# opherlieber/rltime

Hardware: AMD Instinct MI355X
Metric: sampled transitions/sec (= learner steps/sec x B x T), IQN-LSTM B=512 T=80 84x84x4 (higher is better)
Workload: dtype f32

## Files before the change

include/mirl.h:

```cpp
#ifndef MIRL_H
#define MIRL_H

#include <stdint.h>

#ifdef __cplusplus
extern "C" {
#endif

#define MIRL_OK 0
#define MIRL_NEED_MORE 1
#define MIRL_ERR_ARG (-1)
#define MIRL_ERR_HIP (-2)
#define MIRL_ERR_STATE (-3)
#define MIRL_ERR_NOGPU (-4)

#define MIRL_MODE_UNIFORM 0
#define MIRL_MODE_PER 1

typedef struct mirl_replay mirl_replay;

typedef struct mirl_replay_config {
  int64_t size;
  int32_t num_envs;
  int32_t env_base;
// ... 124 lines not shown
                      double gamma, double vf_eps, float* targets, void* stream);

int mirl_loss_dqn(int64_t M, int32_t A, const float* q, const int64_t* actions,
                  const float* targets, const float* weights, double kappa, int32_t mode,
                  double row_scale, float* row_loss, float* dq, float* td, void* stream);
int mirl_loss_iqn(int64_t M, int32_t N, int32_t Nt, int32_t A, const float* z,
                  const float* taus, const int64_t* actions, const float* targets,
                  const float* weights, double kappa, double row_scale,
                  float* row_loss, float* dz, float* abs_td, void* stream);

int mirl_q_target_c51(int64_t M, int32_t A, int32_t Z, const float* logits_target, const float* logits_select,
                      const float* support, const float* returns, const float* nsteps, const float* masks,
                      double gamma, double vmin, double vmax, double delta_z, int32_t projection,
                      float* targets, void* stream);
int mirl_loss_c51(int64_t M, int32_t A, int32_t Z, const float* logits, const int64_t* actions,
                  const float* targets, const float* weights, int32_t mode, double kappa, double row_scale,
                  float* row_loss, float* dlogits, float* report, void* stream);

int mirl_lstm_cell_fwd(int32_t B, int32_t H, float* gates, const float* c_in, const float* keep_next,
                       float* h_out, float* c_out, float* h_next, float* c_next, void* stream);
int mirl_lstm_seq_supported(int32_t T, int32_t B, int32_t H);
int mirl_lstm_seq_workspace_bytes(int32_t B, int32_t H, int64_t* bytes);
int mirl_lstm_seq_fwd(int32_t T, int32_t B, int32_t H, float* gx, const float* w_hh, const float* h0,
                      const float* c0, const float* keep, float* out, float* c_all, float* hm, float* cm,
                      float* h_last, float* c_last, int32_t save_gates, void* workspace, void* stream);
int mirl_lstm_seq_status(int32_t* status);
int mirl_lstm_seq_fwd_grid(int32_t B, int32_t H, int32_t* workgroups, int64_t* lds_bytes, int32_t* compute_units,
                           int32_t* per_compute_unit);
int mirl_lstm_seq_bwd_supported(int32_t T, int32_t B, int32_t H);
int mirl_lstm_seq_bwd_workspace_bytes(int32_t B, int32_t H, int64_t* bytes);
int mirl_lstm_seq_bwd(int32_t T, int32_t B, int32_t H, float* gates, const float* w_hh, const float* c_all,
                      const float* cm, const float* d_out, const float* keep, void* workspace, void* stream);
int mirl_lstm_cell_bwd(int32_t B, int32_t H, float* gates, const float* c_t, const float* c_in,
                       const float* d_out, const float* dh_rec, float* dc_rec, const float* keep_next,
                       int32_t first, void* stream);

int mirl_frames_to_f32_nhwc(int64_t N, int32_t C, int32_t HW, const uint8_t* src, float scale,
                            float* dst, void* stream);
int mirl_frames_to_f32_nhwc_ex(int64_t N, int32_t C, int32_t HW, const uint8_t* src, float scale,
                               float* dst, int32_t per_wg, int32_t flags, void* stream);

int mirl_conv1_u8_supported(int32_t C, int32_t H, int32_t W, int32_t F, int32_t K, int32_t S);
int mirl_conv1_u8_wpk_floats(int64_t* out);
int mirl_conv1_bf16_set(int32_t mode);
int mirl_conv1_wrw_bf16_set(int32_t mode);
int mirl_conv1_u8_fwd(int64_t N, int32_t H, int32_t W, const uint8_t* x, const float* weight,
                      int64_t ws_o, int64_t ws_c, int64_t ws_h, int64_t ws_w, const float* bias,
                      float scale, float* wpk, float* y, void* stream);
int mirl_conv1_u8_fwd_ex(int64_t N, int32_t H, int32_t W, const uint8_t* x, const float* weight,
                         int64_t ws_o, int64_t ws_c, int64_t ws_h, int64_t ws_w, const float* bias,
                         float scale, float* wpk, float* y, int32_t flags, void* stream);

int mirl_conv1_u8_wrw_scratch_floats(int64_t* out);
int mirl_conv1_u8_wrw(int64_t N, int32_t H, int32_t W, const uint8_t* x, const float* g, float scale,
                      float* scratch, float* dw, int64_t ws_o, int64_t ws_c, int64_t ws_h, int64_t ws_w,
                      void* stream);
int mirl_conv1_u8_wrw_ex(int64_t N, int32_t H, int32_t W, const uint8_t* x, const float* g, float scale,
                         float* scratch, float* dw, int64_t ws_o, int64_t ws_c, int64_t ws_h, int64_t ws_w,
                         int32_t flags, void* stream);
int mirl_conv1_u8_wrw_masked(int64_t N, int32_t H, int32_t W, const uint8_t* x, const float* dy, const float* y, float scale,
                             float* scratch, float* dw, int64_t ws_o, int64_t ws_c, int64_t ws_h, int64_t ws_w,
                             float* db, void* stream);

int mirl_conv2_bwd_data_supported(int32_t C, int32_t F, int32_t K, int32_t S, int32_t IH, int32_t IW,
                                  int32_t OH, int32_t OW);
int mirl_conv2_bwd_data(int64_t N, int32_t OH, int32_t OW, const float* g, const float* weight,
                        int64_t ws_o, int64_t ws_c, int64_t ws_h, int64_t ws_w, float* wpk, float* dx,
                        void* stream);
int mirl_conv2_bwd_data_wpk_floats(int64_t* floats);
int mirl_conv2_bwd_data_ex(int64_t N, int32_t OH, int32_t OW, const float* g, const float* weight, int64_t ws_o,
                           int64_t ws_c, int64_t ws_h, int64_t ws_w, float* wpk, int64_t wpk_floats, float* dx, int32_t pipe,
                           void* stream);
int mirl_conv3_bwd_data_supported(int32_t C, int32_t F, int32_t K, int32_t S, int32_t IH, int32_t IW, int32_t OH, int32_t OW);
int mirl_conv3_bwd_data_wpk_floats(int64_t* floats);
int mirl_conv3_bwd_data(int64_t N, int32_t OH, int32_t OW, const float* g, const float* weight, int64_t ws_o,
                        int64_t ws_c, int64_t ws_h, int64_t ws_w, float* wpk, int64_t wpk_floats, float* dx, void* stream);

int mirl_gemm3_supported(int32_t layout, int64_t M, int64_t N, int64_t K);
int mirl_gemm3_workspace_bytes(int32_t layout, int64_t M, int64_t N, int64_t K, int64_t* bytes);
int mirl_gemm3(int32_t layout, int64_t M, int64_t N, int64_t K, const float* A, int64_t lda,
               const float* B, int64_t ldb, float* C, int64_t ldc, const float* bias, int32_t relu,
               void* workspace, int64_t workspace_bytes, void* stream);
int mirl_gemm3_mid_set(int32_t mode);
int mirl_gemm3_nt_mul(int64_t M, int64_t N, int64_t K, const float* A, int64_t lda, const float* B,
                      int64_t ldb, float* C, int64_t ldc, const float* bias, int32_t relu,
                      const float* mul, int64_t ldmul, int32_t group_shift, float* pre, int64_t ldpre,
                      void* stream);
int mirl_gemm3_head_workspace_bytes(int64_t M, int64_t N, int64_t* bytes);
int mirl_gemm3_nt_head(int64_t M, int64_t N, int64_t K, const float* A, int64_t lda, const float* B, int64_t ldb,
                       float* C, int64_t ldc, const float* bias, int32_t relu, const float* w2, int32_t O,
                       const float* bias2, float* out2, int64_t ldo, void* workspace, int64_t workspace_bytes, void* stream);
int mirl_gemm3_nn_qp_partial_rows(int64_t M, int64_t* rows);
int mirl_gemm3_nn_qp(int64_t M, int64_t N, int64_t K, const float* A, int64_t lda, const float* B, int64_t ldb,
                     const float* emb, int64_t ldemb, const float* x, int64_t ldx, float* d_pre, int64_t ldd,
                     float* dx, int64_t lddx, float* db_partial, void* stream);

int mirl_conv3_fwd_supported(int32_t C, int32_t F, int32_t KH, int32_t KW, int32_t S, int32_t H, int32_t W);
int mirl_conv3_fwd(int64_t N, int32_t H, int32_t W, int32_t C, int32_t F, int32_t KH, int32_t KW, int32_t S,
                   const float* x, const float* w, const float* bias, int32_t relu, float* y, void* stream);

int mirl_conv_wrw_b3_supported(int32_t C, int32_t F, int32_t KH, int32_t KW, int32_t S, int32_t H, int32_t W);
int mirl_conv_wrw_b3_scratch_bytes(int32_t C, int32_t F, int32_t KH, int32_t KW, int64_t* bytes);
int mirl_conv_wrw_b3(int64_t N, int32_t H, int32_t W, int32_t C, int32_t F, int32_t KH, int32_t KW, int32_t S,
                     const float* x, const float* g, void* scratch, int64_t scratch_bytes, float* dw, void* stream);

int mirl_bias_relu_rows(int64_t rows, int32_t C, float* y, const float* bias, void* stream);
int mirl_colsum_blocks(int64_t rows, int32_t C, int32_t* blocks);
int mirl_relu_bwd_bias_rows(int64_t rows, int32_t C, const float* dy, const float* y, float* g,
                            float* db, float* partial, int32_t blocks, void* stream);
int mirl_cos_embed(int64_t rows, int32_t D, const float* tau, const float* freq, float* phi, void* stream);
int mirl_cos_embed_rng(int64_t rows, int32_t D, uint64_t seed, const uint64_t* step, const float* freq,
                       float* phi, float* tau_out, void* stream);
int mirl_iqn_mul_fwd(int64_t M, int32_t N, int32_t C, const float* x, const float* emb, float* out, void* stream);
int mirl_iqn_mul_bwd(int64_t M, int32_t N, int32_t C, const float* g, const float* emb, const float* x,
                     float* d_pre, float* dx, float* db, float* partial, int32_t blocks, void* stream);

int mirl_dueling_tail_bwd(int64_t M, int32_t H1, int32_t Hv, int32_t A, int32_t Q, const float* ga,
                          const float* gv, const float* wo, const float* wq, const float* both,
                          float* g, float* db, float* partial, int32_t blocks, void* stream);
int mirl_dueling_tail_bwd_w(int64_t M, int32_t H1, int32_t Hv, int32_t A, int32_t Q, const float* ga,
                            const float* gv, const float* wo, const float* wq, const float* both, float* g,
                            float* db, float* partial, int32_t blocks, float* dwj, float* partial_w,
                            void* stream);

int mirl_actor_head(int32_t E, int32_t N, int32_t A, const float* adv, const float* val, int32_t Q,
                    const double* eps, const double* expo, double eps_min, const float* u, const int64_t* rnd,
                    int32_t* actions, float* qvalues, float* eps_used, void* stream);
int mirl_actor_head_rng(int32_t E, int32_t N, int32_t A, const float* adv, int32_t adv_pitch, const float* val, int32_t Q,
                        const double* eps, const double* expo, double eps_min, uint64_t rng_seed,
                        const uint64_t* rng_step, int32_t* actions, float* qvalues, float* eps_used, void* stream);
int mirl_actor_head_c51(int32_t E, int32_t A, int32_t Z, const float* adv, int32_t adv_pitch, const float* val,
                        int32_t val_pitch, const float* support, const double* eps, const double* expo, double eps_min,
                        const float* u, const int64_t* rnd, uint64_t rng_seed, const uint64_t* rng_step,
                        int32_t* actions, float* qvalues, float* eps_used, void* stream);
int mirl_stack_shift(int32_t E, int32_t P, int32_t plane_bytes, const uint8_t* in, uint8_t* out,
                     const uint8_t* newest, const uint8_t* dones, void* stream);
#define MIRL_STEP_ADVANCE (~0ull)
int mirl_actor_pre(int32_t E, int32_t H, int32_t A, const float* rewards_raw, const uint8_t* dones,
                   const int32_t* actions, const float* h, const float* c, float* xh_tail, int64_t xh_pitch,
                   float* c_in, float* state_pack, float* initials, float* rewards_out, uint8_t* dones_out,
                   int32_t clip_rewards, float* ep_reward, int32_t* ep_len, float* out_reward, int32_t* out_len,
                   int32_t* action_counts, uint64_t* rng_step, uint64_t step, void* stream);
int mirl_synth_env_step(int32_t E, int64_t frame_bytes, const uint8_t* pool, int32_t pool_n, uint64_t* clock, int32_t slot,
                        uint64_t seed, float p_neg, float p_nonpos, float p_done, uint8_t* obs, float* rewards,
                        uint8_t* dones, void* stream);
int mirl_act_conv_supported(int32_t layer, int32_t Ci, int32_t Co, int32_t k, int32_t stride, int32_t Hi, int32_t Wi);
int mirl_act_conv_fwd(int32_t layer, int64_t frames, int32_t Hi, int32_t Wi, const float* x, const float* w_taps,
                      const float* bias, float* y, int64_t y_frame_pitch, void* stream);
int mirl_act_lstm_supported(int32_t E, int32_t H, int32_t K);
int mirl_act_lstm_workspace_bytes(int32_t E, int32_t H, int32_t K, int64_t* bytes);
int mirl_act_lstm_fwd(int32_t E, int32_t H, int32_t K, const float* xh, int64_t xh_pitch, const float* w, const float* bias,
                      const float* c_in, float* h_out, float* c_out, void* workspace, void* stream);
int mirl_act_embed(int32_t E, int32_t N, int32_t H, int32_t D, const float* h, const float* freq, const float* taus,
                   uint64_t seed, const uint64_t* step, const float* wq, const float* bq, float* x, float* tau_out, void* stream);
int mirl_act_head_supported(int32_t E, int32_t N, int32_t H, int32_t D, int32_t HID, int32_t NO);
int mirl_act_head_parts(int32_t HID, int32_t NO, int32_t* parts, int32_t* pitch);
int mirl_act_head_hidden(int32_t R, int32_t H, int32_t HID, int32_t NO, const float* x, const float* wfc, const float* bfc,
                         const float* wout, float* part, void* stream);
int mirl_act_head_select(int32_t E, int32_t N, int32_t A, int32_t parts, int32_t pitch, const float* part, const float* bout,
                         int32_t has_val, const double* eps, const double* expo, double eps_min, uint64_t rng_seed,
                         const uint64_t* rng_step, int32_t* actions, float* qvalues, void* stream);
int mirl_synth_env_step_pre(int32_t E, int64_t frame_bytes, const uint8_t* pool, int32_t pool_n, uint64_t* clock, int32_t slot,
                            uint64_t seed, float p_neg, float p_nonpos, float p_done, uint8_t* obs, float* rewards,
                            uint8_t* dones, int32_t H, int32_t A, const int32_t* actions, const float* h, const float* c,
                            float* xh_tail, int64_t xh_pitch, float* c_in, float* state_pack, float* initials,
                            float* rewards_out, uint8_t* dones_out, int32_t clip_rewards, float* ep_reward, int32_t* ep_len,
// ... 54 lines not shown
```

rltime_amd/_lib.py:

```python
import ctypes as C
import os

import torch

_HERE = os.path.dirname(os.path.abspath(__file__))
LIB_PATH = os.path.join(_HERE, "librltime_hip.so")

MIRL_OK = 0
MIRL_NEED_MORE = 1
MODE_UNIFORM = 0
MODE_PER = 1
INT32_MIN = -2 ** 31


MIRL_OK, MIRL_ERR_ARG, MIRL_ERR_HIP, MIRL_ERR_STATE, MIRL_ERR_NOGPU = 0, -1, -2, -3, -4


class MirlError(RuntimeError):
    code = None


class ReplayConfig(C.Structure):
    _fields_ = [
        ("size", C.c_int64),
# ... 45 lines not shown


class Batch(C.Structure):
    _fields_ = [
        ("frames", C.c_void_p),
        ("extra", C.c_void_p),
        ("state", C.c_void_p),
        ("initials", C.c_void_p),
        ("returns", C.c_void_p),
        ("nsteps", C.c_void_p),
        ("masks", C.c_void_p),
        ("actions", C.c_void_p),
        ("policy", C.c_void_p),
        ("weights", C.c_void_p),
        ("loss_indices", C.c_void_p),
    ]


def _load():
    if not os.path.isfile(LIB_PATH):
        raise MirlError(
            "%s not found: build it with `python -c 'import __graft_entry__ as g; "
            "g.build()'` (rltime_amd/csrc/build.sh). rltime_amd has no CPU "
            "fallback." % LIB_PATH)
    lib = C.CDLL(LIB_PATH)
    lib.mirl_last_error.restype = C.c_char_p
    return lib


lib = _load()

_vp, _i32, _i64, _u64, _f64 = C.c_void_p, C.c_int32, C.c_int64, C.c_uint64, C.c_double
_P = C.POINTER

_SIGNATURES = {
    "mirl_device_count": [],
    "mirl_replay_create": [_P(ReplayConfig), _P(_vp)],
    "mirl_replay_destroy": [_vp],
    "mirl_replay_ingest": [_vp, _P(Ingest), _vp],
    "mirl_replay_ingest_plan": [_vp, _i32, _i32, _vp, _vp],
    "mirl_replay_ingest_planned": [_vp, _i32, _P(Ingest), _vp],
    "mirl_ingest_fused_set": [_i32],
    "mirl_replay_prime_stack": [_vp, _vp, _i64, _vp],
    "mirl_replay_needed_feed_count": [_vp, _i32, _i32, _P(_i64)],
    "mirl_replay_sample": [_vp, _i32, _f64, _vp, _u64, _vp, _vp, _vp, _vp, _vp, _vp, _vp],
    "mirl_replay_sample_ready": [_vp, _i32, _P(_i32)],
    "mirl_replay_sample_skip": [_vp, _i32],
    "mirl_replay_tree_root": [_vp, _vp, _vp],
    "mirl_replay_sample_global": [_vp, _i32, _i32, _i32, _i32, _i32, _vp, _f64, _u64, _vp, _vp, _vp, _vp, _vp, _vp, _vp, _vp],
    "mirl_replay_profile": [_vp, _i32, _P(_i64), _P(_f64)],
    "mirl_profile_set": [_i32],
    "mirl_profile_collect": [_P(_i32)],
    "mirl_profile_get": [_i32, C.c_char_p, _i32, _P(_i64), _P(_f64), _P(_f64)],
    "mirl_profile_get_flop": [_i32, _vp],
    "mirl_profile_reset": [],
    "mirl_replay_save": [_vp, C.c_char_p],
    "mirl_replay_load": [_vp, C.c_char_p],
    "mirl_replay_uniform_total": [_vp, _P(_i64)],
    "mirl_replay_set_train_quota": [_vp, _i64],
    "mirl_replay_state_rows": [_vp, _P(_i32), _P(_i32)],
    "mirl_replay_gather": [_vp, _i32, _vp, _vp, _vp, _vp, _P(Batch), _vp],
    "mirl_replay_update_losses": [_vp, _i64, _vp, _vp, _vp],
    "mirl_replay_stats": [_vp, _P(_i64), _P(_i64), _P(_i64), _P(_i64), _P(_i64)],
    "mirl_replay_env_meta": [_vp, _vp, _vp],
    "mirl_replay_free_slots": [_vp, _vp, _P(_i64)],
    "mirl_replay_slot_table": [_vp, _vp, _vp],
    "mirl_replay_tree_nodes": [_vp, _vp, _vp, _vp],
    "mirl_replay_tree_set_leaves": [_vp, _i64, _vp, _vp, _vp],
    "mirl_replay_tree_find": [_vp, _i32, _vp, _vp, _vp],
    "mirl_replay_losses_peek": [_vp, _i32, _i64, _i32, _vp],
    "mirl_q_target_dqn": [_i64, _i32, _vp, _vp, _vp, _vp, _vp, _f64, _f64, _vp, _vp],
    "mirl_q_target_iqn": [_i64, _i32, _i32, _i32, _vp, _vp, _vp, _vp, _vp, _f64, _f64, _vp, _vp],
    "mirl_loss_dqn": [_i64, _i32, _vp, _vp, _vp, _vp, _f64, _i32, _f64, _vp, _vp, _vp, _vp],
    "mirl_loss_iqn": [_i64, _i32, _i32, _i32, _vp, _vp, _vp, _vp, _vp, _f64, _f64, _vp, _vp, _vp, _vp],
    "mirl_q_target_c51": [_i64, _i32, _i32, _vp, _vp, _vp, _vp, _vp, _vp, _f64, _f64, _f64, _f64, _i32, _vp, _vp],
    "mirl_loss_c51": [_i64, _i32, _i32, _vp, _vp, _vp, _vp, _i32, _f64, _f64, _vp, _vp, _vp, _vp],
    "mirl_actor_head_c51": [_i32, _i32, _i32, _vp, _i32, _vp, _i32, _vp, _vp, _vp, _f64, _vp, _vp, _u64, _vp, _vp, _vp, _vp, _vp],
    "mirl_lstm_cell_fwd": [_i32, _i32, _vp, _vp, _vp, _vp, _vp, _vp, _vp, _vp],
    "mirl_lstm_seq_supported": [_i32, _i32, _i32],
    "mirl_lstm_seq_workspace_bytes": [_i32, _i32, _P(_i64)],
    "mirl_lstm_seq_fwd": [_i32, _i32, _i32, _vp, _vp, _vp, _vp, _vp, _vp, _vp, _vp, _vp, _vp, _vp, _i32, _vp, _vp],
    "mirl_lstm_seq_status": [_P(_i32)],
    "mirl_gemm3_mid_set": [_i32],
    "mirl_lstm_seq_fwd_grid": [_i32, _i32, _P(_i32), _P(_i64), _P(_i32), _P(_i32)],
    "mirl_lstm_seq_bwd_supported": [_i32, _i32, _i32],
    "mirl_lstm_seq_bwd_workspace_bytes": [_i32, _i32, _P(_i64)],
    "mirl_lstm_seq_bwd": [_i32, _i32, _i32, _vp, _vp, _vp, _vp, _vp, _vp, _vp, _vp],
    "mirl_lstm_cell_bwd": [_i32, _i32, _vp, _vp, _vp, _vp, _vp, _vp, _vp, _i32, _vp],
    "mirl_frames_to_f32_nhwc": [_i64, _i32, _i32, _vp, C.c_float, _vp, _vp],
    "mirl_frames_to_f32_nhwc_ex": [_i64, _i32, _i32, _vp, C.c_float, _vp, _i32, _i32, _vp],
    "mirl_conv1_u8_supported": [_i32, _i32, _i32, _i32, _i32, _i32],
    "mirl_conv1_bf16_set": [_i32],
    "mirl_conv1_wrw_bf16_set": [_i32],
    "mirl_conv1_u8_wpk_floats": [_P(_i64)],
    "mirl_conv1_u8_fwd": [_i64, _i32, _i32, _vp, _vp, _i64, _i64, _i64, _i64, _vp, C.c_float, _vp, _vp, _vp],
    "mirl_conv1_u8_fwd_ex": [_i64, _i32, _i32, _vp, _vp, _i64, _i64, _i64, _i64, _vp, C.c_float, _vp, _vp, _i32, _vp],
    "mirl_conv1_u8_wrw_scratch_floats": [_P(_i64)],
    "mirl_conv1_u8_wrw_ex": [_i64, _i32, _i32, _vp, _vp, C.c_float, _vp, _vp, _i64, _i64, _i64, _i64, _i32, _vp],
    "mirl_conv1_u8_wrw_masked": [_i64, _i32, _i32, _vp, _vp, _vp, C.c_float, _vp, _vp, _i64, _i64, _i64, _i64, _vp, _vp],
    "mirl_conv1_u8_wrw": [_i64, _i32, _i32, _vp, _vp, C.c_float, _vp, _vp, _i64, _i64, _i64, _i64, _vp],
    "mirl_conv2_bwd_data_supported": [_i32, _i32, _i32, _i32, _i32, _i32, _i32, _i32],
    "mirl_conv2_bwd_data": [_i64, _i32, _i32, _vp, _vp, _i64, _i64, _i64, _i64, _vp, _vp, _vp],
    "mirl_conv2_bwd_data_wpk_floats": [_P(_i64)],
    "mirl_conv3_bwd_data_supported": [_i32, _i32, _i32, _i32, _i32, _i32, _i32, _i32],
    "mirl_conv3_bwd_data_wpk_floats": [_P(_i64)],
    "mirl_conv3_bwd_data": [_i64, _i32, _i32, _vp, _vp, _i64, _i64, _i64, _i64, _vp, _i64, _vp, _vp],
    "mirl_conv2_bwd_data_ex": [_i64, _i32, _i32, _vp, _vp, _i64, _i64, _i64, _i64, _vp, _i64, _vp, _i32, _vp],
    "mirl_conv3_fwd_supported": [_i32, _i32, _i32, _i32, _i32, _i32, _i32],
    "mirl_conv3_fwd": [_i64, _i32, _i32, _i32, _i32, _i32, _i32, _i32, _vp, _vp, _vp, _i32, _vp, _vp],
    "mirl_conv_wrw_b3_supported": [_i32, _i32, _i32, _i32, _i32, _i32, _i32],
    "mirl_conv_wrw_b3_scratch_bytes": [_i32, _i32, _i32, _i32, _P(_i64)],
    "mirl_conv_wrw_b3": [_i64, _i32, _i32, _i32, _i32, _i32, _i32, _i32, _vp, _vp, _vp, _i64, _vp, _vp],
    "mirl_gemm3_supported": [_i32, _i64, _i64, _i64],
    "mirl_gemm3_workspace_bytes": [_i32, _i64, _i64, _i64, _P(_i64)],
    "mirl_gemm3": [_i32, _i64, _i64, _i64, _vp, _i64, _vp, _i64, _vp, _i64, _vp, _i32, _vp, _i64, _vp],
    "mirl_gemm3_nt_mul": [_i64, _i64, _i64, _vp, _i64, _vp, _i64, _vp, _i64, _vp, _i32, _vp, _i64, _i32, _vp, _i64, _vp],
    "mirl_gemm3_nn_qp_partial_rows": [_i64, _P(_i64)],
    "mirl_gemm3_nn_qp": [_i64, _i64, _i64, _vp, _i64, _vp, _i64, _vp, _i64, _vp, _i64, _vp, _i64, _vp, _i64, _vp, _vp],
    "mirl_gemm3_head_workspace_bytes": [_i64, _i64, _P(_i64)],
    "mirl_gemm3_nt_head": [_i64, _i64, _i64, _vp, _i64, _vp, _i64, _vp, _i64, _vp, _i32, _vp, _i32, _vp, _vp, _i64, _vp, _i64, _vp],
    "mirl_act_conv_supported": [_i32, _i32, _i32, _i32, _i32, _i32, _i32],
    "mirl_act_conv_fwd": [_i32, _i64, _i32, _i32, _vp, _vp, _vp, _vp, _i64, _vp],
    "mirl_act_lstm_supported": [_i32, _i32, _i32],
    "mirl_act_lstm_workspace_bytes": [_i32, _i32, _i32, _P(_i64)],
    "mirl_act_lstm_fwd": [_i32, _i32, _i32, _vp, _i64, _vp, _vp, _vp, _vp, _vp, _vp, _vp],
    "mirl_act_embed": [_i32, _i32, _i32, _i32, _vp, _vp, _vp, _u64, _vp, _vp, _vp, _vp, _vp, _vp],
    "mirl_act_head_supported": [_i32, _i32, _i32, _i32, _i32, _i32],
    "mirl_act_head_parts": [_i32, _i32, _P(_i32), _P(_i32)],
    "mirl_act_head_hidden": [_i32, _i32, _i32, _i32, _vp, _vp, _vp, _vp, _vp, _vp],
    "mirl_act_head_select": [_i32, _i32, _i32, _i32, _i32, _vp, _vp, _i32, _vp, _vp, _f64, _u64, _vp, _vp, _vp, _vp],
    "mirl_bias_relu_rows": [_i64, _i32, _vp, _vp, _vp],
    "mirl_colsum_blocks": [_i64, _i32, _P(_i32)],
    "mirl_relu_bwd_bias_rows": [_i64, _i32, _vp, _vp, _vp, _vp, _vp, _i32, _vp],
    "mirl_cos_embed": [_i64, _i32, _vp, _vp, _vp, _vp],
    "mirl_cos_embed_rng": [_i64, _i32, _u64, _vp, _vp, _vp, _vp, _vp],
    "mirl_adam_clip_workspace_bytes": [_i32, _vp, _vp],
    "mirl_adam_clip_step": [_i32, _vp, _vp, _vp, _vp, _vp, _vp, _f64, _vp, _f64, _f64, _f64, _f64, _vp, _i64, _vp, _vp],
    "mirl_adam_clip_step_guarded": [_i32, _vp, _vp, _vp, _vp, _vp, _vp, _f64, _vp, _f64, _f64, _f64, _f64, _vp, _i64, _vp, _vp, _vp],
    "mirl_step_guard_open": [_vp, _vp, _i64, _vp, _i32, _vp],
    "mirl_replay_update_losses_guarded": [_vp, _i64, _vp, _vp, _vp, _vp],
    "mirl_lstm_seq_status_device": [_P(_vp)],
    "mirl_iqn_mul_fwd": [_i64, _i32, _i32, _vp, _vp, _vp, _vp],
    "mirl_iqn_mul_bwd": [_i64, _i32, _i32, _vp, _vp, _vp, _vp, _vp, _vp, _vp, _i32, _vp],
    "mirl_dueling_tail_bwd": [_i64, _i32, _i32, _i32, _i32, _vp, _vp, _vp, _vp, _vp, _vp, _vp, _vp, _i32, _vp],
    "mirl_dueling_tail_bwd_w": [_i64, _i32, _i32, _i32, _i32, _vp, _vp, _vp, _vp, _vp, _vp, _vp, _vp, _i32, _vp, _vp, _vp],
    "mirl_actor_head": [_i32, _i32, _i32, _vp, _vp, _i32, _vp, _vp, _f64, _vp, _vp, _vp, _vp, _vp, _vp],
    "mirl_actor_head_rng": [_i32, _i32, _i32, _vp, _i32, _vp, _i32, _vp, _vp, _f64, _u64, _vp, _vp, _vp, _vp, _vp],
    "mirl_stack_shift": [_i32, _i32, _i32, _vp, _vp, _vp, _vp, _vp],
    "mirl_synth_env_step": [_i32, _i64, _vp, _i32, _vp, _i32, _u64, C.c_float, C.c_float, C.c_float, _vp, _vp, _vp, _vp],
    "mirl_synth_env_step_pre": [_i32, _i64, _vp, _i32, _vp, _i32, _u64, C.c_float, C.c_float, C.c_float, _vp, _vp, _vp,
                                _i32, _i32, _vp, _vp, _vp, _vp, _i64, _vp, _vp, _vp, _vp, _vp, _i32, _vp, _vp, _vp, _vp, _vp, _vp, _u64, _vp],
    "mirl_actor_pre": [_i32, _i32, _i32, _vp, _vp, _vp, _vp, _vp, _vp, _i64, _vp, _vp, _vp, _vp, _vp, _i32, _vp, _vp, _vp, _vp,
                       _vp, _vp, _u64, _vp],
    "mirl_episode_track": [_i32, _i32, _vp, _vp, _vp, _vp, _vp, _vp, _vp, _vp, _vp],
    "mirl_copy_bytes": [_vp, _vp, _i64, _vp],
    "mirl_copy_bytes_ex": [_vp, _vp, _i64, _i32, _vp],
    "mirl_book_create": [_P(ReplayConfig), _P(_vp)],
    "mirl_book_destroy": [_vp],
    "mirl_book_ingest": [_vp, _i32, _vp],
    "mirl_book_stats": [_vp, _P(_i64), _P(_i64), _P(_i64), _P(_i64), _P(_i64)],
    "mirl_book_env_meta": [_vp, _vp, _vp],
    "mirl_book_free_slots": [_vp, _vp, _P(_i64)],
    "mirl_book_slot_table": [_vp, _vp, _vp],
    "mirl_book_needed_feed_count": [_vp, _i32, _i32, _P(_i64)],
    "mirl_book_charge_quota": [_vp, _i32],
    "mirl_book_uniform_total": [_vp, _P(_i64)],
# ... 61 lines not shown
```

rltime_amd/csrc/gemm3.hip:

```cpp
#include "common.hpp"
#include "split3.hpp"
#include <stdlib.h>

namespace mirl {

struct G3Args {
  const float* A; const float* B; float* C; const float* bias;
  int64_t M, N, K;
  int64_t lda, ldb, ldc;
  int relu;
  int mt, nt;
  int splits;
  int steps_per_split;
  const float* mul; int64_t ldmul; int mul_shift;
  float* pre; int64_t ldpre;
  int vec_ok;
  const float* w2; float* part;
  float* gsum; int64_t ldgsum;
};


template <bool KC>
struct G3Loader {
  const float* p[2];
// ... 389 lines not shown
  const int b_lds = rb * G3_PITCH + kq * 8;
  float va[2][4], vb[4];
  auto load_b = [&]() { const float4 q = *reinterpret_cast<const float4*>(pb); vb[0] = q.x; vb[1] = q.y; vb[2] = q.z; vb[3] = q.w; pb += 16; };
  auto store_b = [&](char* planes) {
    uint2 h, m, lo;
    g3_split4(vb, h, m, lo);
    *reinterpret_cast<uint2*>(planes + b_lds) = h;
    *reinterpret_cast<uint2*>(planes + G3M_BPLANE + b_lds) = m;
    *reinterpret_cast<uint2*>(planes + 2 * G3M_BPLANE + b_lds) = lo;
  };
  const int a_off = (wm * 128 + (lane & 31)) * G3_PITCH + (lane >> 5) * 16;
  const int b_off = (wn * 32 + (lane & 31)) * G3_PITCH + (lane >> 5) * 16;
  const bool stage_first = (wu >> 2) & 1;

  g3_f32x16 acc[4];
#pragma unroll
  for (int i = 0; i < 4; ++i)
#pragma unroll
    for (int r = 0; r < 16; ++r) acc[i][r] = 0.0f;
  constexpr int PA[6] = {2, 0, 1, 1, 0, 0};
  constexpr int PB[6] = {0, 2, 1, 0, 1, 0};

  if (nk > 0) { la.load(va); load_b(); la.store(g3_lds, va); store_b(g3_lds + 3 * G3_PLANE); }
  if (nk > 1) { la.load(va); load_b(); }
  g3_barrier();
  for (int64_t k = 0; k < nk; ++k) {
    const char* cur = g3_lds + (k & 1) * G3M_STAGE;
    char* nxt = g3_lds + ((k + 1) & 1) * G3M_STAGE;
    if (stage_first) {
      if (k + 1 < nk) { la.store(nxt, va); store_b(nxt + 3 * G3_PLANE); }
      if (k + 2 < nk) { la.load(va); load_b(); }
    }
    {
      const char* pa = cur + a_off;
      const char* pbf = cur + 3 * G3_PLANE + b_off;
      g3_bf16x8 bf[3];
#pragma unroll
      for (int p = 0; p < 3; ++p) bf[p] = *reinterpret_cast<const g3_bf16x8*>(pbf + p * G3M_BPLANE);
      __builtin_amdgcn_s_setprio(1);
#pragma unroll
      for (int ih = 0; ih < 2; ++ih) {
        g3_bf16x8 a[3][2];
#pragma unroll
        for (int p = 0; p < 3; ++p)
#pragma unroll
          for (int i = 0; i < 2; ++i) a[p][i] = *reinterpret_cast<const g3_bf16x8*>(pa + p * G3_PLANE + (ih * 2 + i) * 32 * G3_PITCH);
#pragma unroll
        for (int c = 0; c < 6; ++c)
#pragma unroll
          for (int i = 0; i < 2; ++i) acc[ih * 2 + i] = g3_mfma(a[PA[c]][i], bf[PB[c]], acc[ih * 2 + i]);
      }
      __builtin_amdgcn_s_setprio(0);
    }
    if (!stage_first) {
      if (k + 1 < nk) { la.store(nxt, va); store_b(nxt + 3 * G3_PLANE); }
      if (k + 2 < nk) { la.load(va); load_b(); }
    }
    g3_barrier();
  }

  float* tl = reinterpret_cast<float*>(g3_lds) + wu * (32 * G3M_EPITCH);
  const int c4 = lane & 7;
  const int64_t col = n0 + wn * 32 + c4 * 4;
  float4 bv = make_float4(0.f, 0.f, 0.f, 0.f);
  if (g.bias && col < g.N) bv = *reinterpret_cast<const float4*>(g.bias + col);
#pragma unroll
  for (int i = 0; i < 4; ++i) {
#pragma unroll
    for (int r = 0; r < 16; ++r)
      tl[((r & 3) + 8 * (r >> 2) + 4 * (lane >> 5)) * G3M_EPITCH + (lane & 31)] = acc[i][r];
    asm volatile("s_waitcnt lgkmcnt(0)" ::: "memory");
#pragma unroll
    for (int q = 0; q < 4; ++q) {
      const int rl = q * 8 + (lane >> 3);
      const int64_t row = m0 + wm * 128 + i * 32 + rl;
      float4 v = *reinterpret_cast<const float4*>(tl + rl * G3M_EPITCH + c4 * 4);
      if (row < g.M && col < g.N) {
        v.x += bv.x; v.y += bv.y; v.z += bv.z; v.w += bv.w;
        if (g.relu) { v.x = v.x > 0.f ? v.x : 0.f; v.y = v.y > 0.f ? v.y : 0.f; v.z = v.z > 0.f ? v.z : 0.f; v.w = v.w > 0.f ? v.w : 0.f; }
        *reinterpret_cast<float4*>(g.C + row * g.ldc + col) = v;
      }
    }
    asm volatile("s_waitcnt lgkmcnt(0)" ::: "memory");
  }
}

__global__ void __launch_bounds__(256)
k_gemm3_reduce(const float* __restrict__ partial, int splits, int64_t M, int64_t N, float* __restrict__ out, int64_t ldc) {
  const int64_t n4 = N >> 2;
  const int64_t total = M * n4;
  for (int64_t i = (int64_t)blockIdx.x * blockDim.x + threadIdx.x; i < total; i += (int64_t)gridDim.x * blockDim.x) {
    const int64_t row = i / n4, c4 = i - row * n4;
    float4 s = make_float4(0.f, 0.f, 0.f, 0.f);
    for (int k = 0; k < splits; ++k) {
      const float4 v = *reinterpret_cast<const float4*>(partial + ((int64_t)k * M + row) * N + c4 * 4);
      s.x += v.x; s.y += v.y; s.z += v.z; s.w += v.w;
    }
    *reinterpret_cast<float4*>(out + row * ldc + c4 * 4) = s;
  }
}

__global__ void __launch_bounds__(256)
k_g3_head_reduce(const float* __restrict__ part, int ncb, int64_t M, int O, const float* __restrict__ bias2,
                 float* __restrict__ out, int64_t ldo) {
  for (int64_t i = (int64_t)blockIdx.x * 256 + threadIdx.x; i < M * 2; i += (int64_t)gridDim.x * 256) {
    const int64_t row = i >> 1;
    const int half = (int)(i & 1);
    float4 sum = make_float4(0.f, 0.f, 0.f, 0.f);
    for (int cb = 0; cb < ncb; ++cb) {
      const float4 v = *reinterpret_cast<const float4*>(part + ((int64_t)cb * M + row) * 8 + half * 4);
      sum.x += v.x; sum.y += v.y; sum.z += v.z; sum.w += v.w;
    }
    const float r[4] = {sum.x, sum.y, sum.z, sum.w};
#pragma unroll
    for (int e = 0; e < 4; ++e) {
      const int o = half * 4 + e;
      if (o < O) out[row * ldo + o] = r[e] + (bias2 ? bias2[o] : 0.f);
    }
  }
}

static int g_g3_mid_mode = -1;

static int g3_splits(int64_t M, int64_t N, int64_t K) {
  const int64_t tiles = ((M + 255) / 256) * ((N + 255) / 256);
  int64_t s = 8 * ((256 + 8 * tiles - 1) / (8 * tiles));
  const int64_t nk = K / 16;
  while (s > 8 && nk / s < 64) s -= 8;
  return (int)s;
}

}

extern "C" int mirl_gemm3_supported(int32_t layout, int64_t M, int64_t N, int64_t K) {
  if (layout < 0 || layout > 2) return 0;
  if (M < 1 || N < 1 || K < 16 || (K % 16)) return 0;
  if (M >= (1LL << 31) || N >= (1LL << 31)) return 0;
  if (layout == 2) {
    if (N % 4) return 0;
    if (K / 16 < 8) return 0;
  }
  return 1;
}

extern "C" int mirl_gemm3_workspace_bytes(int32_t layout, int64_t M, int64_t N, int64_t K, int64_t* bytes) {
  using namespace mirl;
  if (!bytes) return fail(MIRL_ERR_ARG, "gemm3_workspace_bytes: null out");
  if (!mirl_gemm3_supported(layout, M, N, K)) return fail(MIRL_ERR_ARG, "gemm3: unsupported layout / shape");
  *bytes = layout == 2 ? (int64_t)g3_splits(M, N, K) * M * N * (int64_t)sizeof(float) : 0;
  return MIRL_OK;
}

static int g3_launch(int32_t layout, int64_t M, int64_t N, int64_t K, const float* A, int64_t lda, const float* B,
                     int64_t ldb, float* C, int64_t ldc, const float* bias, int32_t relu, void* workspace,
                     int64_t workspace_bytes, const float* mul, int64_t ldmul, int32_t mul_shift, float* pre, int64_t ldpre,
                     void* stream, const float* w2 = nullptr, float* part = nullptr,
                     float* gsum = nullptr, int64_t ldgsum = 0) {
  using namespace mirl;
  if (!mirl_gemm3_supported(layout, M, N, K)) return fail(MIRL_ERR_ARG, "gemm3: unsupported layout / shape");
  if (!A || !B || (!C && !w2)) return fail(MIRL_ERR_ARG, "gemm3: null operand");
  const bool akc = layout != 2, bkc = layout == 0;
  if (akc && ((lda % 4) || ((uintptr_t)A % 16) || lda < K)) return fail(MIRL_ERR_ARG, "gemm3: A must be 16-byte aligned with lda % 4 == 0");
  if (bkc && ((ldb % 4) || ((uintptr_t)B % 16) || ldb < K)) return fail(MIRL_ERR_ARG, "gemm3: B must be 16-byte aligned with ldb % 4 == 0");
  if (!akc && lda < M) return fail(MIRL_ERR_ARG, "gemm3: lda < M");
  if (!bkc && ldb < N) return fail(MIRL_ERR_ARG, "gemm3: ldb < N");
  if (ldc < N) return fail(MIRL_ERR_ARG, "gemm3: ldc < N");
// ... 12 lines not shown
  if (K <= 128) {
    int dev = 0, cus = 256;
    (void)hipGetDevice(&dev);
    (void)hipDeviceGetAttribute(&cus, hipDeviceAttributeMultiprocessorCount, dev);
    const unsigned resident = (unsigned)(cus / 8 * 8);
    if (grid > resident) grid = resident;
  }
  if (layout == 2) {
    g.splits = g3_splits(M, N, K);
    const int64_t need = (int64_t)g.splits * M * N * (int64_t)sizeof(float);
    if (!workspace || workspace_bytes < need || ((uintptr_t)workspace % 16) || (ldc % 4) || ((uintptr_t)C % 16))
      return fail(MIRL_ERR_ARG, "gemm3: split-K workspace too small / misaligned");
    g.steps_per_split = (int)((K / 16 + g.splits - 1) / g.splits);
    g.C = (float*)workspace; g.ldc = N;
    grid = (unsigned)(g.mt * g.nt * g.splits);
  }
  const int vec = g.vec_ok ? 1 : 0;
  if (g_g3_mid_mode != 0 && layout == 0 && !mul && !w2 && !gsum && vec && (N % 4) == 0 && (int64_t)g.mt * g.nt < 192 && N > 128 &&
      ((int64_t)g.mt * ((N + G3M_BROWS - 1) / G3M_BROWS) >= 192 || (int64_t)g.mt * g.nt < 24)) {
    static bool mid_attr = false;
    if (!mid_attr) { MIRL_HIP(hipFuncSetAttribute((const void*)k_gemm3_mid, hipFuncAttributeMaxDynamicSharedMemorySize, G3M_LDS)); mid_attr = true; }
    g.nt = (int)((N + G3M_BROWS - 1) / G3M_BROWS);
    const unsigned mgrid = (unsigned)(8 * ((g.mt + 7) / 8) * g.nt);
    ProfScope ps("k_gemm3_nt_mid", 4.0 * ((double)M * K + (double)N * K + (double)M * N), st, 2.0 * (double)M * (double)N * (double)K);
    void* kargs[] = {(void*)&g};
    MIRL_HIP(hipLaunchKernel((const void*)k_gemm3_mid, dim3(mgrid), dim3(512), kargs, G3M_LDS, st));
    return MIRL_OK;
  }
  static bool attr[4][2] = {{false, false}, {false, false}, {false, false}, {false, false}};
  const void* fns[4][2] = {{(const void*)k_gemm3<true, true, 0, false>, (const void*)k_gemm3<true, true, 0, true>},
                           {(const void*)k_gemm3<true, false, 0, false>, (const void*)k_gemm3<true, false, 0, true>},
                           {nullptr , (const void*)k_gemm3<false, false, 0, true>},
                           {(const void*)k_gemm3<true, true, 1, false>, (const void*)k_gemm3<true, true, 1, true>}};
  const int which = (mul && !gsum) ? 3 : layout;
  const void* fn = fns[which][vec];
  if (gsum) {
    if (!vec || layout != 1 || !mul || mul_shift != 5 || !pre || !part || (ldgsum % 4) || ((uintptr_t)gsum % 16) || ((uintptr_t)part % 16) || (M % 32))
      return fail(MIRL_ERR_ARG, "gemm3: the fused feature-product backward needs the NN form, groups of 32 rows and 16-byte aligned rows");
    static bool qp_attr = false;
    fn = (const void*)k_gemm3<true, false, 3, true>;
    if (!qp_attr) { MIRL_HIP(hipFuncSetAttribute(fn, hipFuncAttributeMaxDynamicSharedMemorySize, G3_LDS)); qp_attr = true; }
  } else if (w2) {
    if (!vec || layout != 0 || mul || !part) return fail(MIRL_ERR_ARG, "gemm3: the fused following layer needs the NT form with 16-byte aligned rows");
    static bool hd_attr = false;
    fn = (const void*)k_gemm3<true, true, 2, true>;
    if (!hd_attr) { MIRL_HIP(hipFuncSetAttribute(fn, hipFuncAttributeMaxDynamicSharedMemorySize, G3_LDS)); hd_attr = true; }
  } else if (layout == 2 && N <= 64) {
    static bool nr_attr = false;
    fn = (const void*)k_gemm3<false, false, 0, true, true>;
    if (!nr_attr) { MIRL_HIP(hipFuncSetAttribute(fn, hipFuncAttributeMaxDynamicSharedMemorySize, G3_LDS)); nr_attr = true; }
  } else
  if (!attr[which][vec]) { MIRL_HIP(hipFuncSetAttribute(fn, hipFuncAttributeMaxDynamicSharedMemorySize, G3_LDS)); attr[which][vec] = true; }
  {
    const double flop = 2.0 * (double)M * (double)N * (double)K;
    double bytes = 4.0 * ((double)M * K + (double)N * K + (double)M * N * (layout == 2 ? (double)g.splits : 1.0));
    if (mul) bytes += 4.0 * ((pre ? (double)M * N : 0.0) + (double)(M >> mul_shift) * N * (gsum ? 2.0 : 1.0));
    if (w2) bytes += 4.0 * (8.0 * (double)N + 8.0 * (double)M * (double)((N + 63) / 64)) - (C ? 0.0 : 4.0 * (double)M * N);
    ProfScope ps(gsum ? "k_gemm3_nn_qp" : mul ? "k_gemm3_nt_mul" : w2 ? "k_gemm3_nt_head" : layout == 0 ? "k_gemm3_nt" : layout == 1 ? "k_gemm3_nn" : "k_gemm3_tn", bytes, st, flop);
    void* kargs[] = {(void*)&g};
    MIRL_HIP(hipLaunchKernel(fn, dim3(grid), dim3(512), kargs, G3_LDS, st));
  }
  if (layout == 2) {
    ProfScope ps("k_gemm3_reduce", (double)(g.splits + 1) * (double)M * (double)N * 4.0, st);
    const int64_t total = M * (N / 4);
    unsigned rg = (unsigned)((total + 255) / 256); if (rg > 4096) rg = 4096;
    hipLaunchKernelGGL(k_gemm3_reduce, dim3(rg), dim3(256), 0, st, (const float*)workspace, g.splits, M, N, C, ldc);
    MIRL_LAUNCH_CHECK();
  }
  return MIRL_OK;
}

extern "C" int mirl_gemm3(int32_t layout, int64_t M, int64_t N, int64_t K, const float* A, int64_t lda, const float* B,
                          int64_t ldb, float* C, int64_t ldc, const float* bias, int32_t relu, void* workspace,
                          int64_t workspace_bytes, void* stream) {
  return g3_launch(layout, M, N, K, A, lda, B, ldb, C, ldc, bias, relu, workspace, workspace_bytes, nullptr, 0, 0, nullptr, 0, stream);
}

extern "C" int mirl_gemm3_mid_set(int32_t mode) {
  if (mode < -1 || mode > 1) return mirl::fail(MIRL_ERR_ARG, "gemm3_mid_set: mode is -1 (default), 0 or 1");
  mirl::g_g3_mid_mode = mode;
  return MIRL_OK;
}

extern "C" int mirl_gemm3_nt_mul(int64_t M, int64_t N, int64_t K, const float* A, int64_t lda, const float* B, int64_t ldb,
                                 float* C, int64_t ldc, const float* bias, int32_t relu, const float* mul, int64_t ldmul,
                                 int32_t group_shift, float* pre, int64_t ldpre, void* stream) {
  using namespace mirl;
  if (!mul || group_shift < 0 || group_shift > 30 || ldmul < N || (pre && ldpre < N))
    return fail(MIRL_ERR_ARG, "gemm3_nt_mul: bad multiplier / pre-activation arguments");
  return g3_launch(0, M, N, K, A, lda, B, ldb, C, ldc, bias, relu, nullptr, 0, mul, ldmul, group_shift, pre, ldpre, stream);
}

extern "C" int mirl_gemm3_nn_qp_partial_rows(int64_t M, int64_t* rows) {
  if (!rows || M < 1) return mirl::fail(MIRL_ERR_ARG, "gemm3_nn_qp_partial_rows: M >= 1");
  *rows = 2 * ((M + 255) / 256);
  return MIRL_OK;
}

extern "C" int mirl_gemm3_nn_qp(int64_t M, int64_t N, int64_t K, const float* A, int64_t lda, const float* B, int64_t ldb,
                                const float* emb, int64_t ldemb, const float* x, int64_t ldx, float* d_pre, int64_t ldd,
                                float* dx, int64_t lddx, float* db_partial, void* stream) {
  using namespace mirl;
  if (!emb || !x || !d_pre || !dx || !db_partial || ldemb < N || ldx < N || lddx < N || (ldemb % 4) || ((uintptr_t)emb % 16))
    return fail(MIRL_ERR_ARG, "gemm3_nn_qp: bad embedding / feature / output arguments");
  return g3_launch(1, M, N, K, A, lda, B, ldb, d_pre, ldd, nullptr, 0, nullptr, 0, x, ldx, 5, const_cast<float*>(emb), ldemb, stream,
                   nullptr, db_partial, dx, lddx);
}

extern "C" int mirl_gemm3_head_workspace_bytes(int64_t M, int64_t N, int64_t* bytes) {
  if (!bytes || M < 1 || N < 1) return mirl::fail(MIRL_ERR_ARG, "bad gemm3_head_workspace_bytes arguments");
  *bytes = 8 * (int64_t)sizeof(float) * M * ((N + 255) / 256 * 4);
  return MIRL_OK;
}

extern "C" int mirl_gemm3_nt_head(int64_t M, int64_t N, int64_t K, const float* A, int64_t lda, const float* B, int64_t ldb,
                                  float* C, int64_t ldc, const float* bias, int32_t relu, const float* w2, int32_t O,
                                  const float* bias2, float* out2, int64_t ldo, void* workspace, int64_t workspace_bytes,
                                  void* stream) {
  using namespace mirl;
  int64_t need = 0;
  if (O < 1 || O > 8 || !w2 || !out2 || ldo < O || !workspace || mirl_gemm3_head_workspace_bytes(M, N, &need) || workspace_bytes < need ||
      ((uintptr_t)workspace % 16) || (N % 4))
    return fail(MIRL_ERR_ARG, "bad gemm3_nt_head arguments (1 <= O <= 8, N % 4 == 0, 16-byte aligned workspace of head_workspace_bytes)");
  if (!C) ldc = N;
  int rc = g3_launch(0, M, N, K, A, lda, B, ldb, C, ldc, bias, relu, nullptr, 0, nullptr, 0, 0, nullptr, 0, stream, w2,
                     (float*)workspace);
  if (rc) return rc;
  const int ncb = (int)((N + 255) / 256 * 4);
  hipStream_t st = (hipStream_t)stream;
  ProfScope ps("k_g3_head_reduce", 4.0 * (8.0 * ncb + O) * (double)M, st);
  unsigned grid = (unsigned)((2 * M + 255) / 256); if (grid > 16384) grid = 16384;
  hipLaunchKernelGGL(k_g3_head_reduce, dim3(grid), dim3(256), 0, st, (const float*)workspace, ncb, M, (int)O, bias2, out2, ldo);
  MIRL_LAUNCH_CHECK();
  return MIRL_OK;
}
```

Baseline: 480,700.

## Add row-streaming K=64 gemm kernel for nt_mul with LDS-resident B

Adds a dedicated kernel for the IQN embedding gemm (K=64, N multiple of 32). It keeps the bf16x3-split B matrix resident in LDS for a column range and streams 32-row A blocks per wave, with XCD-aware block mapping. The multiplier row is hoisted once per block when the group is 32 rows or larger, and outputs use nontemporal stores. The aim is to avoid re-splitting and reloading B tiles and the split-K/tiling overhead of the generic gemm3 path. The cost is heavy LDS use per block and a larger code surface, and any shape that fails the checks falls back to the old path.

```diff
diff --git a/include/mirl.h b/include/mirl.h
--- a/include/mirl.h
+++ b/include/mirl.h
@@ -230,6 +230,10 @@
                const float* B, int64_t ldb, float* C, int64_t ldc, const float* bias, int32_t relu,
                void* workspace, int64_t workspace_bytes, void* stream);
 int mirl_gemm3_mid_set(int32_t mode);
+int mirl_gemm3_qrow_set(int32_t mode);
+int mirl_gemm3_nt_mul_path(int64_t M, int64_t N, int64_t K, const float* A, int64_t lda, const float* B, int64_t ldb,
+                           const float* C, int64_t ldc, const float* bias, const float* mul, int64_t ldmul,
+                           const float* pre, int64_t ldpre);
 int mirl_gemm3_nt_mul(int64_t M, int64_t N, int64_t K, const float* A, int64_t lda, const float* B,
                       int64_t ldb, float* C, int64_t ldc, const float* bias, int32_t relu,
                       const float* mul, int64_t ldmul, int32_t group_shift, float* pre, int64_t ldpre,
diff --git a/rltime_amd/_lib.py b/rltime_amd/_lib.py
--- a/rltime_amd/_lib.py
+++ b/rltime_amd/_lib.py
@@ -151,6 +151,8 @@
     "mirl_lstm_seq_fwd": [_i32, _i32, _i32, _vp, _vp, _vp, _vp, _vp, _vp, _vp, _vp, _vp, _vp, _vp, _i32, _vp, _vp],
     "mirl_lstm_seq_status": [_P(_i32)],
     "mirl_gemm3_mid_set": [_i32],
+    "mirl_gemm3_qrow_set": [_i32],
+    "mirl_gemm3_nt_mul_path": [_i64, _i64, _i64, _vp, _i64, _vp, _i64, _vp, _i64, _vp, _vp, _i64, _vp, _i64],
     "mirl_lstm_seq_fwd_grid": [_i32, _i32, _P(_i32), _P(_i64), _P(_i32), _P(_i32)],
     "mirl_lstm_seq_bwd_supported": [_i32, _i32, _i32],
     "mirl_lstm_seq_bwd_workspace_bytes": [_i32, _i32, _P(_i64)],
diff --git a/rltime_amd/csrc/gemm3.hip b/rltime_amd/csrc/gemm3.hip
--- a/rltime_amd/csrc/gemm3.hip
+++ b/rltime_amd/csrc/gemm3.hip
@@ -495,6 +495,159 @@
       }
     }
     asm volatile("s_waitcnt lgkmcnt(0)" ::: "memory");
+  }
+}
+
+constexpr int QR_WAVES = 16;
+constexpr int QR_COLS = 256;
+constexpr int QR_BPITCH = 144;
+constexpr int QR_BPLANE = QR_COLS * QR_BPITCH;
+constexpr int QR_TFLOATS = 16 * 32;
+constexpr int QR_T_OFF = 3 * QR_BPLANE;
+constexpr int QR_BIAS_OFF = QR_T_OFF + QR_WAVES * QR_TFLOATS * 4;
+constexpr int QR_MUL_OFF = QR_BIAS_OFF + QR_COLS * 4;
+constexpr int QR_LDS = QR_MUL_OFF + QR_WAVES * QR_COLS * 4;
+
+struct QRowArgs {
+  const float* A; const float* B; float* C; const float* bias; const float* mul; float* pre;
+  int64_t M, lda, ldb, ldc, ldmul, ldpre;
+  int64_t blocks;
+  int N, relu, mul_shift;
+  int ranges;
+  int range_tiles;
+  int streams;
+};
+
+__device__ __forceinline__ g3_bf16x8 qr_frag(uint2 a, uint2 b) {
+  const uint4 u = make_uint4(a.x, a.y, b.x, b.y);
+  return __builtin_bit_cast(g3_bf16x8, u);
+}
+
+template <bool HOIST>
+__global__ void __launch_bounds__(1024)
+k_gemm3_qrow(QRowArgs g) {
+  extern __shared__ __attribute__((aligned(16))) char g3_lds[];
+  const int t = threadIdx.x, lane = t & 63;
+  const int wu = __builtin_amdgcn_readfirstlane(t >> 6);
+  const int b = blockIdx.x, xcd = b & 7, l = b >> 3;
+  const int range = l % g.ranges, stream = (l / g.ranges) * 8 + xcd;
+  if (stream >= g.streams) return;
+  const int n0 = range * g.range_tiles * 32;
+  int ncols = g.N - n0; if (ncols > g.range_tiles * 32) ncols = g.range_tiles * 32;
+  if (ncols <= 0) return;
+  const int ntiles = ncols >> 5;
+
+  {
+    const int r = t >> 2, kq = t & 3;
+    if (r < ncols) {
+      const float* src = g.B + (int64_t)(n0 + r) * g.ldb + kq * 16;
+      float4 q[4];
+#pragma unroll
+      for (int e = 0; e < 4; ++e) q[e] = *reinterpret_cast<const float4*>(src + 4 * e);
+      char* d = g3_lds + r * QR_BPITCH + kq * 32;
+#pragma unroll
+      for (int e = 0; e < 4; ++e) {
+        const float v[4] = {q[e].x, q[e].y, q[e].z, q[e].w};
+        uint2 h, m, lo;
+        g3_split4(v, h, m, lo);
+        *reinterpret_cast<uint2*>(d + e * 8) = h;
+        *reinterpret_cast<uint2*>(d + QR_BPLANE + e * 8) = m;
+        *reinterpret_cast<uint2*>(d + 2 * QR_BPLANE + e * 8) = lo;
+      }
+    }
+    if (t < QR_COLS) reinterpret_cast<float*>(g3_lds + QR_BIAS_OFF)[t] = (g.bias && t < ncols) ? g.bias[n0 + t] : 0.f;
+  }
+  g3_barrier();
+
+  float* tl = reinterpret_cast<float*>(g3_lds + QR_T_OFF) + wu * QR_TFLOATS;
+  float* ml = reinterpret_cast<float*>(g3_lds + QR_MUL_OFF) + wu * QR_COLS;
+  const float* bl = reinterpret_cast<const float*>(g3_lds + QR_BIAS_OFF);
+  const int frow = lane & 31, kg = lane >> 5;
+  const char* bfrag = g3_lds + frow * QR_BPITCH + kg * 16;
+  const int c4 = lane & 7, rq = lane >> 3;
+  constexpr int PA[6] = {2, 0, 1, 1, 0, 0};
+  constexpr int PB[6] = {0, 2, 1, 0, 1, 0};
+
+  for (int64_t blk = (int64_t)stream * QR_WAVES + wu; blk < g.blocks; blk += (int64_t)g.streams * QR_WAVES) {
+    const int64_t m0 = blk * 32;
+    g3_bf16x8 a[4][3];
+    {
+      int64_t arow = m0 + frow; if (arow > g.M - 1) arow = g.M - 1;
+      const float* pa = g.A + arow * g.lda + kg * 8;
+      float4 q[4][2];
+#pragma unroll
+      for (int s = 0; s < 4; ++s)
+#pragma unroll
+        for (int e = 0; e < 2; ++e) q[s][e] = *reinterpret_cast<const float4*>(pa + 16 * s + 4 * e);
+      if (HOIST) {
+        float4 mv = make_float4(0.f, 0.f, 0.f, 0.f);
+        if (lane * 4 < ncols) mv = *reinterpret_cast<const float4*>(g.mul + (m0 >> g.mul_shift) * g.ldmul + n0 + lane * 4);
+        *reinterpret_cast<float4*>(ml + lane * 4) = mv;
+      }
+#pragma unroll
+      for (int s = 0; s < 4; ++s) {
+        const float v0[4] = {q[s][0].x, q[s][0].y, q[s][0].z, q[s][0].w};
+        const float v1[4] = {q[s][1].x, q[s][1].y, q[s][1].z, q[s][1].w};
+        uint2 h0, m0_, l0, h1, m1, l1;
+        g3_split4(v0, h0, m0_, l0);
+        g3_split4(v1, h1, m1, l1);
+        a[s][0] = qr_frag(h0, h1); a[s][1] = qr_frag(m0_, m1); a[s][2] = qr_frag(l0, l1);
+      }
+    }
+
+#pragma unroll 1
+    for (int j = 0; j < ntiles; ++j) {
+      const int cl = j * 32 + c4 * 4;
+      const int64_t col = n0 + cl;
+      g3_f32x16 acc;
+#pragma unroll
+      for (int r = 0; r < 16; ++r) acc[r] = 0.0f;
+      const char* pb = bfrag + j * 32 * QR_BPITCH;
+#pragma unroll
+      for (int s = 0; s < 4; ++s) {
+        g3_bf16x8 bf[3];
+#pragma unroll
+        for (int p = 0; p < 3; ++p) bf[p] = *reinterpret_cast<const g3_bf16x8*>(pb + p * QR_BPLANE + s * 32);
+#pragma unroll
+        for (int c = 0; c < 6; ++c) acc = g3_mfma(a[s][PA[c]], bf[PB[c]], acc);
+      }
+
+      const float4 bv = *reinterpret_cast<const float4*>(bl + cl);
+      float4 mg[2][2];
+      if (HOIST) {
+        mg[0][0] = *reinterpret_cast<const float4*>(ml + cl);
+      } else {
+#pragma unroll
+        for (int h = 0; h < 2; ++h)
+#pragma unroll
+          for (int q = 0; q < 2; ++q) {
+            int64_t row = m0 + h * 16 + q * 8 + rq; if (row > g.M - 1) row = g.M - 1;
+            mg[h][q] = *reinterpret_cast<const float4*>(g.mul + (row >> g.mul_shift) * g.ldmul + col);
+          }
+      }
+
+#pragma unroll
+      for (int h = 0; h < 2; ++h) {
+#pragma unroll
+        for (int rr = 0; rr < 8; ++rr) tl[((rr & 3) + 8 * (rr >> 2) + 4 * kg) * 32 + frow] = acc[8 * h + rr];
+        asm volatile("s_waitcnt lgkmcnt(0)" ::: "memory");
+#pragma unroll
+        for (int q = 0; q < 2; ++q) {
+          const int rl = q * 8 + rq;
+          const int64_t row = m0 + h * 16 + rl;
+          float4 v = *reinterpret_cast<const float4*>(tl + rl * 32 + c4 * 4);
+          if (row < g.M) {
+            v.x += bv.x; v.y += bv.y; v.z += bv.z; v.w += bv.w;
+            if (g.relu) { v.x = v.x > 0.f ? v.x : 0.f; v.y = v.y > 0.f ? v.y : 0.f; v.z = v.z > 0.f ? v.z : 0.f; v.w = v.w > 0.f ? v.w : 0.f; }
+            if (g.pre) __builtin_nontemporal_store(g3_f32x4{v.x, v.y, v.z, v.w}, reinterpret_cast<g3_f32x4*>(g.pre + row * g.ldpre + col));
+            const float4 m = HOIST ? mg[0][0] : mg[h][q];
+            v.x *= m.x; v.y *= m.y; v.z *= m.z; v.w *= m.w;
+            __builtin_nontemporal_store(g3_f32x4{v.x, v.y, v.z, v.w}, reinterpret_cast<g3_f32x4*>(g.C + row * g.ldc + col));
+          }
+        }
+        asm volatile("s_waitcnt lgkmcnt(0)" ::: "memory");
+      }
+    }
   }
 }
 
@@ -673,12 +826,67 @@
   return MIRL_OK;
 }
 
+static int g_g3_qrow_mode = -1;
+
+static int g3_qrow_path(int64_t M, int64_t N, int64_t K, const float* A, int64_t lda, const float* B, int64_t ldb, const float* C,
+                        int64_t ldc, const float* bias, const float* mul, int64_t ldmul, const float* pre, int64_t ldpre) {
+  if (g_g3_qrow_mode == 0) return 0;
+  if (K != 64 || M < 1 || N < 32 || (N % 32)) return 0;
+  if (lda < 64 || ldb < 64 || (lda % 4) || (ldb % 4) || ((uintptr_t)A % 16) || ((uintptr_t)B % 16)) return 0;
+  if ((ldc % 4) || ((uintptr_t)C % 16) || ((uintptr_t)bias % 16) || (ldmul % 4) || ((uintptr_t)mul % 16)) return 0;
+  if (pre && ((ldpre % 4) || ((uintptr_t)pre % 16))) return 0;
+  return 1;
+}
+
+extern "C" int mirl_gemm3_qrow_set(int32_t mode) {
+  if (mode < -1 || mode > 1) return mirl::fail(MIRL_ERR_ARG, "gemm3_qrow_set: mode is -1 (default), 0 or 1");
+  g_g3_qrow_mode = mode;
+  return MIRL_OK;
+}
+
+extern "C" int mirl_gemm3_nt_mul_path(int64_t M, int64_t N, int64_t K, const float* A, int64_t lda, const float* B, int64_t ldb,
+                                      const float* C, int64_t ldc, const float* bias, const float* mul, int64_t ldmul,
+                                      const float* pre, int64_t ldpre) {
+  return g3_qrow_path(M, N, K, A, lda, B, ldb, C, ldc, bias, mul, ldmul, pre, ldpre);
+}
+
 extern "C" int mirl_gemm3_nt_mul(int64_t M, int64_t N, int64_t K, const float* A, int64_t lda, const float* B, int64_t ldb,
                                  float* C, int64_t ldc, const float* bias, int32_t relu, const float* mul, int64_t ldmul,
                                  int32_t group_shift, float* pre, int64_t ldpre, void* stream) {
   using namespace mirl;
   if (!mul || group_shift < 0 || group_shift > 30 || ldmul < N || (pre && ldpre < N))
     return fail(MIRL_ERR_ARG, "gemm3_nt_mul: bad multiplier / pre-activation arguments");
+  if (A && B && C && ldc >= N && mirl_gemm3_supported(0, M, N, K) &&
+      g3_qrow_path(M, N, K, A, lda, B, ldb, C, ldc, bias, mul, ldmul, pre, ldpre)) {
+    hipStream_t st = (hipStream_t)stream;
+    int dev = 0, cus = 256;
+    (void)hipGetDevice(&dev);
+    (void)hipDeviceGetAttribute(&cus, hipDeviceAttributeMultiprocessorCount, dev);
+    QRowArgs q;
+    q.A = A; q.B = B; q.C = C; q.bias = bias; q.mul = mul; q.pre = pre;
+    q.M = M; q.lda = lda; q.ldb = ldb; q.ldc = ldc; q.ldmul = ldmul; q.ldpre = ldpre;
+    q.blocks = (M + 31) / 32;
+    q.N = (int)N; q.relu = relu ? 1 : 0; q.mul_shift = group_shift;
+    const int tiles = (int)(N / 32);
+    q.ranges = (tiles * 32 + QR_COLS - 1) / QR_COLS;
+    q.range_tiles = (tiles + q.ranges - 1) / q.ranges;
+    q.ranges = (tiles + q.range_tiles - 1) / q.range_tiles;
+    int64_t streams = cus / q.ranges; if (streams < 1) streams = 1;
+    const int64_t want = (q.blocks + QR_WAVES - 1) / QR_WAVES;
+    if (streams > want) streams = want;
+    q.streams = (int)streams;
+    const unsigned grid = (unsigned)(8 * ((q.streams + 7) / 8) * q.ranges);
+    const int hoist = group_shift >= 5 ? 1 : 0;
+    const void* qfn = hoist ? (const void*)k_gemm3_qrow<true> : (const void*)k_gemm3_qrow<false>;
+    static bool qr_attr[2] = {false, false};
+    if (!qr_attr[hoist]) { MIRL_HIP(hipFuncSetAttribute(qfn, hipFuncAttributeMaxDynamicSharedMemorySize, QR_LDS)); qr_attr[hoist] = true; }
+    const double flop = 2.0 * (double)M * (double)N * (double)K;
+    const double bytes = 4.0 * ((double)M * K + (double)N * K + (double)M * N) + 4.0 * ((pre ? (double)M * N : 0.0) + (double)(M >> group_shift) * N);
+    ProfScope ps("k_gemm3_nt_mul", bytes, st, flop);
+    void* kargs[] = {(void*)&q};
+    MIRL_HIP(hipLaunchKernel(qfn, dim3(grid), dim3(QR_WAVES * 64), kargs, QR_LDS, st));
+    return MIRL_OK;
+  }
   return g3_launch(0, M, N, K, A, lda, B, ldb, C, ldc, bias, relu, nullptr, 0, mul, ldmul, group_shift, pre, ldpre, stream);
 }
 
```

Result: no change. 484,100, median of 6 (+0.7%).
